# xl-tang3/RCOT

Measured on AMD Instinct MI355X. Metric: 128x128 patches/sec (gen+critic step), higher is better.
Workload: dtype fp32 (exact fp32 MFMA everywhere); 1 GPU; BASELINE configs[1]: Restormer T_net(decoder=True)+F_net(128), denoise_50, RMSprop, paired, B=8/GPU 128x128; global_batch=8, patch=128, parallelism=dp1, gemm_prec=fp32

## Files before the change

include/rcot_hip.h:

```cpp
#ifndef RCOT_HIP_H
#define RCOT_HIP_H
#include <stddef.h>

#ifdef __cplusplus
extern "C" {
#endif

#define RCOT_ABI_VERSION 39

#define RCOT_PREC_FP32 0
#define RCOT_PREC_BF16X3 1
#define RCOT_PREC_BF16X6 2
#define RCOT_PREC_BF16X1 3

int rcot_abi_version(void);
int rcot_debug_nt_coop(int mask);
int rcot_profile_begin(void);
int rcot_profile_end(char* out, int n);
int rcot_last_kernel(char* out, int n);

int rcot_conv1x1_fwd(const float* W, long ldw, const float* X, long sXb, float* Y, long sYb, int B, int Ci, int Co,
                     int N, const float* ln_mu, const float* ln_rs, const float* ln_w, const float* ln_b,
                     const float* R, long sRb, float beta, void* stream);
int rcot_conv1x1_dgrad(const float* W, long ldw, const float* dY, long sdYb, float* dX, long sdXb, int B, int Ci,
// ... 62 lines not shown
int rcot_conv_pcm_merge(const float* dQ, long ldq, float* dX, int B, int C, int H, int W, void* stream);
int rcot_conv_pcm_pack(const float* W, const int* rowoff, const int* koff, int M, int K, void* Apk, void* stream);
int rcot_conv_pcm(const void* Apk, int M, int K, const float* Xp, long ldb, int N, const int* tapoff, int ntaps, const float* bias,
                  float lrelu, const int* colmap, float* Y, long ldy, float* ws, size_t ws_bytes, void* stream);
int rcot_pixel_shuffle(const float* in, float* out, long planes, int H, int W, int mode, void* stream);

int rcot_ln_stats(const float* x, float* mu, float* rs, int B, int C, int N, void* stream);
int rcot_ln_bwd(const float* g, const float* x, const float* mu, const float* rs, const float* w, const float* dres,
                float* dx, float* dw, float* db, int B, int C, int N, void* ws, long ws_bytes, void* stream);
int rcot_ln_bwd_rows(int B, int C, int N);
int rcot_block_param_reduce(const float* part1, const float* part2, int rows, int C, float* gw1, float* gb1, float* gw2,
                            float* gb2, const float* dWo_part, float* gWo, const float* dtemp_part, float* gtemp, int B,
                            int heads, const long long* slab_sets, int n_sets, void* stream);

int rcot_dwconv3x3(const float* x, const float* w, float* y, int B, int C, int H, int W, int flip, void* stream);
int rcot_gdfn_gate_fwd(const float* p, const float* w, float* g, int B, int hid, int H, int W, void* stream);
int rcot_gdfn_gate_bwd(const float* p, const float* w, const float* dg, float* dd, float* dwg, int B, int hid, int H,
                       int W, void* stream);
int rcot_gdfn_bwd(const float* p, const float* w, const float* dg, float* dp, float* dwg, float* dd_scratch, int B, int hid,
                  int H, int W, void* stream);
int rcot_dwconv3x3_wgrad(const float* dy, const float* x, float* dw, int B, int C, int H, int W, void* stream);
int rcot_dwconv3x3_bwd(const float* dy, const float* x, const float* w, float* dx, float* dwg, int B, int C, int H, int W,
                       void* stream);

int rcot_row_sumsq(const float* x, float* out, int B, int R, int N, long sXb, void* stream);
int rcot_attn_softmax(const float* Graw, int S, int ld, const float* sq, const float* temp, float* Gn, float* A, int B,
                      int heads, int c, void* stream);
int rcot_attn_bwd_small(const float* dA, const float* A, const float* Gn, const float* sq, const float* temp,
                        float* dtemp_part, float* Eq, float* EqT, float* Dq, float* Dk, int B, int heads, int c,
                        void* stream);
int rcot_attn_core_fwd(const float* u, long sUb, const float* temp, const float* WoT, long ldwt, float* sq, float* Gn, float* A,
                       float* MfT, long ldm, long sMb, int B, int heads, int c, int N, float* ws, size_t ws_bytes, void* stream);
int rcot_attn_core_bwd(const float* dM, int S, int ldd, const float* Wo, const float* A, const float* Gn, const float* sq,
                       const float* temp, float* Mf, float* dWo_part, float* dtemp_part, float* Eq, float* EqT, float* Dq, float* Dk, int B,
                       int heads, int c, void* stream);
int rcot_attn_rows_bwd(const float* dM, int S, int ldd, const float* Wo, const float* A, const float* Gn, const float* sq,
                       const float* temp, float* Mf, float* dWo_part, float* dtemp_part, float* Eq, float* EqT, float* Dq, float* Dk, int B,
                       int heads, int c, int group_tiles, void* ws, size_t ws_bytes, void* stream);
int rcot_attn_rows_ws_bytes(int B, int heads, int c, int group_tiles);
int rcot_batch_reduce(const float* src, float* dst, int B, long n, float beta, void* stream);

int rcot_lrelu_bwd(const float* dy, const float* a, float* dz, long n, float slope, void* stream);
int rcot_bias_grad(const float* dz, float* db, int B, int C, int P, void* stream);
int rcot_axpby2d(const float* x, long sx, const float* y, long sy, float* out, long so, long rows, long cols, float a,
                 float b, void* stream);
int rcot_fill(float* p, long n, float v, void* stream);
int rcot_lerp(const float* t, const float* f, const float* alpha, float* out, int B, long per, void* stream);
// ... 97 lines not shown
```

rcot_amd/csrc/attn_core.hip:

```cpp
#include <cstdlib>
#include "gemm_core.h"
#include "../../include/rcot_hip.h"

using namespace rcot;

namespace {

template <int CT>
struct AHead {
    static constexpr int cp = 16 * CT;
    static constexpr int c = CT == 2 ? 24 : cp;
    static constexpr int LDA = (cp % 32 == 16) ? cp : cp + 16;
};

template <int CT>
struct AC : AHead<CT> {
    using AHead<CT>::cp;
    using AHead<CT>::c;
    using AHead<CT>::LDA;
    static constexpr int PX = CT == 6 ? 128 : 256;
    static constexpr int Q4 = PX / 4;
    static constexpr int LDQ = PX + 8;
    static constexpr int NW = CT == 6 ? 8 : 4;
    static constexpr int NT = 64 * NW;
// ... 12 lines not shown
__device__ __forceinline__ void fold_prefetch(float (&bfr)[AC<CT>::MTW][AC<CT>::cp / 4], const float* __restrict__ WoT, long ldwt, int h,
                                              int mt0, int mt1) {
    constexpr int cp = AC<CT>::cp, c = AC<CT>::c, NW = AC<CT>::NW, MTW = AC<CT>::MTW;
    const int lane = threadIdx.x & 63, wave = threadIdx.x >> 6;
    const int r16 = lane & 15, kq = lane >> 4;
#pragma unroll
    for (int t = 0; t < MTW; ++t) {
        const int mt = mt0 + wave + NW * t;
        const float* Wl = WoT + ((long)h * c + kq) * ldwt + 16 * mt + r16;
#pragma unroll
        for (int s = 0; s < cp / 4; ++s) bfr[t][s] = (mt < mt1 && 4 * s + kq < c) ? Wl[(long)(4 * s) * ldwt] : 0.f;
    }
}

template <int CT>
__device__ __forceinline__ void attn_tail(float* Gs, const float* sqs, const float (&bfr)[AC<CT>::MTW][AC<CT>::cp / 4], int h, int b,
                                          int heads, const float* __restrict__ temp, float* __restrict__ Gn,
                                          float* __restrict__ A, float* __restrict__ MfT, long ldm, long sMb, int mt0, int mt1,
                                          bool small_out) {
    constexpr int cp = AC<CT>::cp, c = AC<CT>::c, LDA = AC<CT>::LDA, NW = AC<CT>::NW, NT = AC<CT>::NT, MTW = AC<CT>::MTW;
    const int lane = threadIdx.x & 63, wave = threadIdx.x >> 6;
#ifdef AC_NO_TAIL
    if (sMb != -12345) return;
#endif
    const long off = ((long)b * heads + h) * c * c;
    const float tau = temp[h];
    const int grp = threadIdx.x >> 4, gl = threadIdx.x & 15;
    float kn[CT];
#pragma unroll
    for (int t = 0; t < CT; ++t) kn[t] = gl + 16 * t < c ? clamp_norm(sqs[cp + gl + 16 * t]) : 1.f;
#pragma unroll 1
    for (int i = grp; i < cp; i += NT / 16) {
        float* row = Gs + i * LDA;
        const float nq = clamp_norm(sqs[i]);
        float g[CT], e[CT], mx = -INFINITY, sum = 0.f;
#pragma unroll
// ... 11 lines not shown
        }
#pragma unroll
        for (int o = 8; o > 0; o >>= 1) sum += __shfl_xor(sum, o, 64);
        const float inv = i < c ? 1.0f / sum : 0.f;
#pragma unroll
        for (int t = 0; t < CT; ++t) {
            const int j = gl + 16 * t;
            row[j] = e[t] * inv;
            if (small_out && i < c && j < c) {
                Gn[off + i * c + j] = g[t];
                A[off + i * c + j] = e[t] * inv;
            }
        }
    }
    __syncthreads();
    const int r16 = lane & 15, kq = lane >> 4;
    float* Mh = MfT + (long)b * sMb + (long)h * c * ldm;
#pragma unroll
    for (int t = 0; t < MTW; ++t) {
        const int mt = mt0 + wave + NW * t;
        if (mt >= mt1) break;
#pragma unroll 1
        for (int jt = 0; jt < CT; ++jt) {
            f32x4 acc = {0.f, 0.f, 0.f, 0.f};
            const float* Ga = Gs + kq * LDA + 16 * jt + r16;
#pragma unroll
            for (int s = 0; s < cp / 4; ++s) acc = __builtin_amdgcn_mfma_f32_16x16x4f32(Ga[4 * s * LDA], bfr[t][s], acc, 0, 0, 0);
            float* Md = Mh + (long)(16 * jt + 4 * kq) * ldm + 16 * mt + r16;
#pragma unroll
            for (int r = 0; r < 4; ++r)
                if (16 * jt + 4 * kq + r < c) Md[(long)r * ldm] = acc[r];
        }
    }
}

template <int CT>
__global__ __launch_bounds__(AC<CT>::NT) void qk_stats_kernel(const float* __restrict__ u, long sUb, int heads, int N, int pxw,
                                                              float* __restrict__ gpart, float* __restrict__ sqpart,
                                                              const float* __restrict__ temp, const float* __restrict__ WoT, long ldwt,
                                                              float* __restrict__ sq, float* __restrict__ Gn, float* __restrict__ A,
                                                              float* __restrict__ MfT, long ldm, long sMb) {
    using K = AC<CT>;
    constexpr int cp = K::cp, c = K::c, LDA = K::LDA, PX = K::PX, LDQ = K::LDQ, NW = K::NW, NT = K::NT, Q4 = K::Q4, RPP = K::RPP, KQ = K::KQ;
    extern __shared__ __attribute__((aligned(16))) float sm[];
    float* T = sm;
    float* Gs = T + K::TILE;
    float* sqs = Gs + cp * LDA;
    const int tid = threadIdx.x, lane = tid & 63, wave = tid >> 6;
// ... 181 lines not shown
        RCOT_LAUNCH_CHECK();
        return RCOT_OK;
    }
    const int pxw = N == 256 ? 128 : (N > 16384 && N % 2048 == 0) ? 2048 : ((N > 1024 && N % 512 == 0) ? 512 : 256);
    const int S = N / pxw;
    const size_t Z = (size_t)B * heads;
    const size_t need = Z * S * ((size_t)c * c + 2 * c) * sizeof(float);
    if (!ws || ws_bytes < need) return RCOT_EWORKSPACE;
    float* gpart = ws;
    float* sqpart = ws + Z * S * c * c;
    launch_lds<qk_stats_kernel<CT>>(dim3(S, heads, B), dim3(K::NT), K::smem_stats, st, u, sUb, heads, N, pxw, gpart, sqpart, temp, WoT,
                                    ldwt, sq, Gn, A, MfT, ldm, sMb);
    RCOT_LAUNCH_CHECK();
    RCOT_LAUNCH(softmax_fold_kernel<CT>, dim3(ms, heads, B), dim3(K::NT), K::smem_fold, st, gpart, sqpart, S, heads, temp, WoT,
                       ldwt, sq, Gn, A, MfT, ldm, sMb);
    RCOT_LAUNCH_CHECK();
    return RCOT_OK;
}

template <int CT>
struct AB : AHead<CT> {
    using AHead<CT>::cp;
    using AHead<CT>::c;
    using AHead<CT>::LDA;
    static constexpr int LD = cp + 2;
    static constexpr int NW = 4, NT = 256;
    static constexpr int NEL = (cp * cp + NT - 1) / NT;
    static constexpr int Q4 = c / 4;
    static constexpr int NLD = (16 * Q4 + 63) / 64;
    static_assert(NW * 2 * 16 * LD >= cp * LDA, "Gn is staged in the tile region for the tail");
// ... 512 lines not shown
int rcot_attn_core_fwd(const float* u, long sUb, const float* temp, const float* WoT, long ldwt, float* sq, float* Gn, float* A,
                       float* MfT, long ldm, long sMb, int B, int heads, int c, int N, float* ws, size_t ws_bytes, void* stream) {
    if (!u || !temp || !WoT || !sq || !Gn || !A || !MfT || B <= 0 || heads <= 0 || c <= 0 || N <= 0 || B > 65535 || heads > 65535)
        return RCOT_EINVAL;
    const int C = heads * c;
    if ((reinterpret_cast<uintptr_t>(u) & 15) || (sUb & 3) || ldwt < C || ldm < C) return RCOT_EINVAL;
    if ((C % 16) || (N % 256) || N > 65536) return RCOT_EUNSUPPORTED;
    if (N > 4096 && (N % 512)) return RCOT_EUNSUPPORTED;
    hipStream_t st = (hipStream_t)stream;
    if (c == 48) return launch_core_fwd<3>(u, sUb, temp, WoT, ldwt, sq, Gn, A, MfT, ldm, sMb, B, heads, c, N, ws, ws_bytes, st);
    if (c == 96) return launch_core_fwd<6>(u, sUb, temp, WoT, ldwt, sq, Gn, A, MfT, ldm, sMb, B, heads, c, N, ws, ws_bytes, st);
    if (c == 24) return launch_core_fwd<2>(u, sUb, temp, WoT, ldwt, sq, Gn, A, MfT, ldm, sMb, B, heads, c, N, ws, ws_bytes, st);
    return RCOT_EUNSUPPORTED;
}

int rcot_attn_core_bwd(const float* dM, int S, int ldd, const float* Wo, const float* A, const float* Gn, const float* sq,
                       const float* temp, float* Mf, float* dWo_part, float* dtemp_part, float* Eq, float* EqT, float* Dq, float* Dk, int B,
                       int heads, int c, void* stream) {
    if (!dM || !Wo || !A || !Gn || !sq || !temp || !Mf || !dWo_part || !dtemp_part || !Eq || !EqT || !Dq || !Dk || B <= 0 ||
        heads <= 0 || B > 65535 || heads > 65535 || S < 0 || S > 8)
        return RCOT_EINVAL;
    const int C = heads * c;
    if ((C % 16) || (c != 24 && c != 48 && c != 96)) return RCOT_EUNSUPPORTED;
    if (S == 0) ldd = C;
    if (ldd < C || (ldd & 3) || (reinterpret_cast<uintptr_t>(dM) & 15) || (reinterpret_cast<uintptr_t>(Wo) & 15)) return RCOT_EINVAL;
    const long sDs = (long)C * ldd, sDb = (long)(S < 1 ? 1 : S) * sDs;
    hipStream_t st = (hipStream_t)stream;
    if (c == 48) return launch_core_bwd<3>(dM, S, ldd, sDs, sDb, Wo, A, Gn, sq, temp, Mf, dWo_part, dtemp_part, Eq, EqT, Dq, Dk, B, heads, st);
    if (c == 96) return launch_core_bwd<6>(dM, S, ldd, sDs, sDb, Wo, A, Gn, sq, temp, Mf, dWo_part, dtemp_part, Eq, EqT, Dq, Dk, B, heads, st);
    return launch_core_bwd<2>(dM, S, ldd, sDs, sDb, Wo, A, Gn, sq, temp, Mf, dWo_part, dtemp_part, Eq, EqT, Dq, Dk, B, heads, st);
// ... 35 lines not shown
```

rcot_amd/csrc/stencil.hip:

```cpp
#include <type_traits>
#include "common.h"
#include "../../include/rcot_hip.h"

using namespace rcot;

namespace {

struct Row6 { float v[6]; };
struct Patch { Row6 r[6]; };

__device__ __forceinline__ float from_lane_below(float v) {
    return __builtin_bit_cast(float, __builtin_amdgcn_update_dpp(0, __builtin_bit_cast(int, v), 0x138, 0xf, 0xf, true));
}
__device__ __forceinline__ float from_lane_above(float v) {
    return __builtin_bit_cast(float, __builtin_amdgcn_update_dpp(0, __builtin_bit_cast(int, v), 0x130, 0xf, 0xf, true));
}

__device__ __forceinline__ float keep_bits(float v, int mask) {
    return __builtin_bit_cast(float, __builtin_bit_cast(int, v) & mask);
}

__device__ __forceinline__ void load_row6(const float* __restrict__ plane, int H, int W, int y, int x0, Row6& r) {
    if (y < 0 || y >= H) {
#pragma unroll
// ... 100 lines not shown
    const BlockIdx4 b = block4(q, H, W);
    const int c = (int)(b.plane % C);
    Patch r;
    if (NB) {
        PatchRows rows;
        patch_request(x + b.plane * H * W, H, W, b.y0, b.x0, rows);
        patch_land(rows, H, W, b.y0, b.x0, r);
    } else {
        load_patch(x + b.plane * H * W, H, W, b.y0, b.x0, r);
    }
    float o[4][4];
    stencil16<FLIP>(r, w + c * 9, o);
    float* yp = y + b.plane * H * W + (long)b.y0 * W + b.x0;
#pragma unroll
    for (int i = 0; i < 4; ++i) *reinterpret_cast<float4*>(yp + (long)i * W) = make_float4(o[i][0], o[i][1], o[i][2], o[i][3]);
}

template <bool NB>
__global__ __launch_bounds__(256) void gate_fwd_kernel(const float* __restrict__ p, const float* __restrict__ w,
                                                       float* __restrict__ g, long nblocks, int hid, int H, int W) {
    const long q = (long)blockIdx.x * 256 + threadIdx.x;
    if (q >= nblocks) return;
    const BlockIdx4 b = block4(q, H, W);
    const long bi = b.plane / hid;
    const int j = (int)(b.plane - bi * hid);
    const long hw = (long)H * W;
    const float* p1 = p + (bi * 2 * hid + j) * hw;
    Patch r;
    float d1[4][4], d2[4][4];
    if (NB) {
// ... 422 lines not shown
        RCOT_LAUNCH(dwconv_any_kernel, dim3(grid_for(total)), dim3(256), 0, (hipStream_t)stream, x, w, y, total, C, H, W);
        RCOT_LAUNCH_CHECK();
        return RCOT_OK;
    }
    if (!al16(x) || !al16(y)) return RCOT_EINVAL;
    const long nq = (long)B * C * (H >> 2) * (W >> 2);
    const bool nb = nb_lanes_ok(W);
#define RCOT_DW(F, NB_) do { note_kernel("dwconv_kernel<%s, %s>", tf(F), tf(NB_)); RCOT_LAUNCH((dwconv_kernel<F, NB_>), dim3(cdiv(nq, 256)), dim3(256), 0, (hipStream_t)stream, x, w, y, nq, C, H, W); } while (0)
    if (flip) { if (nb) RCOT_DW(true, true); else RCOT_DW(true, false); }
    else { if (nb) RCOT_DW(false, true); else RCOT_DW(false, false); }
#undef RCOT_DW
    RCOT_LAUNCH_CHECK();
    return RCOT_OK;
}

int rcot_gdfn_gate_fwd(const float* p, const float* w, float* g, int B, int hid, int H, int W, void* stream) {
    if (!p || !w || !g || B <= 0 || hid <= 0 || H <= 0 || W <= 0) return RCOT_EINVAL;
    if ((W & 3) || (H & 3)) {
        const long total = (long)B * hid * H * W;
        note_kernel("gate_fwd_any_kernel");
        RCOT_LAUNCH(gate_fwd_any_kernel, dim3(grid_for(total)), dim3(256), 0, (hipStream_t)stream, p, w, g, total, hid, H, W);
        RCOT_LAUNCH_CHECK();
        return RCOT_OK;
    }
    if (!al16(p) || !al16(g)) return RCOT_EINVAL;
    const long nq = (long)B * hid * (H >> 2) * (W >> 2);
    const bool nb = nb_lanes_ok(W);
    note_kernel("gate_fwd_kernel<%s>", tf(nb));
    if (nb)
        RCOT_LAUNCH(gate_fwd_kernel<true>, dim3(cdiv(nq, 256)), dim3(256), 0, (hipStream_t)stream, p, w, g, nq, hid, H, W);
// ... 82 lines not shown
```

rcot_amd/lib.py:

```python
from __future__ import annotations

import ctypes as C
import os

_HERE = os.path.dirname(os.path.abspath(__file__))
ABI_VERSION = 39
PREC_FP32, PREC_BF16X3, PREC_BF16X6, PREC_BF16X1 = 0, 1, 2, 3
SUMSQ_MAX_PARTS, CB_WORDS = 4096, 16
DECIDE_ADAM0, DECIDE_ADAM1, DECIDE_INHERIT = 1, 2, 4
CB_LR, CB_MAX_NORM, CB_NORM, CB_SCALE, CB_STEPS, CB_CLIPPED, CB_SKIPPED, CB_MAX_SEEN, CB_SKIP, CB_T, CB_BC1, CB_BC2 = 0, 1, 2, 3, 4, 5, 6, 7, 8, 9, 11, 13
LIB_PATH = os.environ.get("RCOT_LIB") or os.path.join(_HERE, "librcot_hip.so")


class RcotLibraryError(RuntimeError):
    pass


class RcotKernelError(RuntimeError):
    pass


_f = C.c_void_p
_l = C.c_long
_i = C.c_int
# ... 37 lines not shown
    "rcot_linear_wgrad": [_f, _f, _f, _i, _i, _i, _fl, _f],
    "rcot_conv2d_fwd": [_f, _f, _f, _f, _i, _i, _i, _i, _i, _i, _i, _i, _i, _fl, _i, _f, _f, _fl, _f, _sz, _f],
    "rcot_conv2d_dgrad": [_f, _f, _f, _i, _i, _i, _i, _i, _i, _i, _i, _i, _fl, _f, _fl, _f, _sz, _f],
    "rcot_conv2d_wgrad": [_f, _f, _f, _i, _i, _i, _i, _i, _i, _i, _i, _i, _fl, _f, _sz, _f],
    "rcot_conv_pcm_prep": [_f, _f, _l, _i, _i, _i, _i, _i, _f],
    "rcot_conv_pcm_wgrad": [_f, _f, _l, _i, _i, _i, _i, _f, _fl, _f, _sz, _i, _f],
    "rcot_conv_pcm_merge": [_f, _l, _f, _i, _i, _i, _i, _f],
    "rcot_conv_pcm_pack": [_f, _f, _f, _i, _i, _f, _f],
    "rcot_conv_pcm": [_f, _i, _i, _f, _l, _i, _f, _i, _f, _fl, _f, _f, _l, _f, _sz, _f],
    "rcot_pixel_shuffle": [_f, _f, _l, _i, _i, _i, _f],
    "rcot_ln_stats": [_f, _f, _f, _i, _i, _i, _f],
    "rcot_ln_bwd": [_f, _f, _f, _f, _f, _f, _f, _f, _f, _i, _i, _i, _f, _l, _f],
    "rcot_ln_bwd_rows": [_i, _i, _i],
    "rcot_block_param_reduce": [_f, _f, _i, _i, _f, _f, _f, _f, _f, _f, _f, _f, _i, _i, _f, _i, _f],
    "rcot_dwconv3x3": [_f, _f, _f, _i, _i, _i, _i, _i, _f],
    "rcot_gdfn_gate_fwd": [_f, _f, _f, _i, _i, _i, _i, _f],
    "rcot_gdfn_gate_bwd": [_f, _f, _f, _f, _f, _i, _i, _i, _i, _f],
    "rcot_gdfn_bwd": [_f, _f, _f, _f, _f, _f, _i, _i, _i, _i, _f],
    "rcot_dwconv3x3_wgrad": [_f, _f, _f, _i, _i, _i, _i, _f],
    "rcot_dwconv3x3_bwd": [_f, _f, _f, _f, _f, _i, _i, _i, _i, _f],
    "rcot_row_sumsq": [_f, _f, _i, _i, _i, _l, _f],
    "rcot_attn_softmax": [_f, _i, _i, _f, _f, _f, _f, _i, _i, _i, _f],
    "rcot_attn_bwd_small": [_f, _f, _f, _f, _f, _f, _f, _f, _f, _f, _i, _i, _i, _f],
    "rcot_attn_core_fwd": [_f, _l, _f, _f, _l, _f, _f, _f, _f, _l, _l, _i, _i, _i, _i, _f, _sz, _f],
    "rcot_attn_core_bwd": [_f, _i, _i] + [_f] * 12 + [_i, _i, _i, _f],
    "rcot_attn_rows_bwd": [_f, _i, _i] + [_f] * 12 + [_i, _i, _i, _i, _f, _sz, _f],
    "rcot_attn_rows_ws_bytes": [_i, _i, _i, _i],
    "rcot_batch_reduce": [_f, _f, _i, _l, _fl, _f],
    "rcot_lrelu_bwd": [_f, _f, _f, _l, _fl, _f],
    "rcot_bias_grad": [_f, _f, _i, _i, _i, _f],
    "rcot_axpby2d": [_f, _l, _f, _l, _f, _l, _l, _l, _fl, _fl, _f],
    "rcot_fill": [_f, _l, _fl, _f],
    "rcot_lerp": [_f, _f, _f, _f, _i, _l, _f],
    "rcot_gp_penalty": [_f, _f, _f, _f, _i, _l, _fl, _f],
    "rcot_ot_reduce": [_f, _f, _f, _f, _i, _l, _f],
    "rcot_fft_plan": [_i, _f, _i],
    "rcot_ot_spectrum": [_f, _f, _f, _f, _f, _f, _sz, _i, _i, _i, _f],
    "rcot_ot_grad": [_f, _f, _f, _f, _f, _f, _f, _f, _f, _i, _l, _fl, _fl, _l, _f],
    "rcot_patch_prep": [_f, _f, _i, _i, _i, _i, _i, _i, _fl, C.c_ulonglong, _f, _f, _f],
# ... 78 lines not shown
```

rcot_amd/net_restormer.py:

```python
from __future__ import annotations

from collections import OrderedDict
from typing import Callable, Dict, List, Optional

import numpy as np

import torch

from . import params as P


class ParamStore:

    def __init__(self, be, shapes, live_order: List[str], dead: List[str]):
        self.be = be
        self.shapes = list(shapes)
        self.layout = P.make_layout(shapes, live_order, dead)
        self.flat = be.zeros(self.layout.n_total)
        self.grad = be.zeros(self.layout.n_total)
        self.p: Dict[str, torch.Tensor] = {}
        self.g: Dict[str, torch.Tensor] = {}
        for name, shp in self.shapes:
            o = self.layout.offset[name]
            n = int(np.prod(shp))
# ... 128 lines not shown
        B, _, H, W = x.shape
        N = H * W
        fast = be.kmajor_worth(C, N, B)
        pstats = wmask is None and getattr(be, "stats_ok", None) is not None and be.stats_ok(C, N, B)
        self.out_stats = None
        t = be.empty(B, 3 * C, H, W)
        if in_stats is not None and pstats:
            mu1, rs1 = in_stats
            be.conv1x1_fwd(self.Wqkv, x, t, ln=(mu1, rs1, self.w1, self.b1), packed=self.pk_qkv)
        else:
            mu1, rs1 = be.empty(B, N), be.empty(B, N)
            be.conv1x1_fwd(self.Wqkv, x, t, ln=(mu1, rs1, self.w1, self.b1), packed=self.pk_qkv, ln_compute=True)
        if wmask is not None:
            t[..., wmask:].zero_()
        u = be.empty(B, 3 * C, H, W)
        be.dwconv3x3(t, self.Wdw, u)
        if wmask is not None:
            u[..., wmask:].zero_()
        sq = be.empty(B, 2 * C)
        Q, K, V = self._qkv_views(u)
        Gn, A, MfT = be.empty(B, hd, c, c), be.empty(B, hd, c, c), be.empty(B, C, C)
        if not be.attn_core_fwd(u, self.temp, self.pk_o[0], sq, Gn, A, MfT):
            be.row_sumsq(u[:, :2 * C], sq)
            Graw = be.bmm_nt_slabs(Q, K)
            if Graw is None:
                Graw = be.empty(B, hd, c, c)
                be.bmm_nt(Q, K, Graw)
            be.attn_softmax(Graw, sq, self.temp, Gn, A)
            be.bmm_nn(A, self._woT_heads(B), MfT.view(B, hd, c, C), transA=True)
        y = be.empty(B, C, H, W)
        mu2, rs2 = be.empty(B, N), be.empty(B, N)
        if fast and pstats:
            be.gemm_kmajor_stats(MfT.unsqueeze(1), V, y.view(B, 1, C, N), C, C, x.view(B, 1, C, N), (mu2, rs2))
        elif fast:
            be.gemm_kmajor(MfT.unsqueeze(1), V, y.view(B, 1, C, N), C, C, R=x.view(B, 1, C, N))
        else:
            be.bmm_nn(MfT.unsqueeze(1), V, y.view(B, 1, C, N), transA=True, R=x.view(B, 1, C, N))
# ... 695 lines not shown
```

rcot_amd/ops.py:

```python
from __future__ import annotations

from typing import Optional, Sequence, Tuple

import os
import struct
import sys

import ctypes as C

import torch

from . import lib as _lib

LN = Optional[Tuple[torch.Tensor, torch.Tensor, torch.Tensor, torch.Tensor]]


ctypes_ll = C.c_longlong


def _ptr(t: Optional[torch.Tensor]):
    return None if t is None else t.data_ptr()


def check_patch_rows(rows, P: int, deg_out, clean_out) -> None:
# ... 841 lines not shown
            self._held_gen[g] = self._held + [dWo_part, dtemp_part]
            self._held = []
            self._side_pending = True
            self._gen ^= 1
            return
        if close_block:
            self.side_join()
        launch()

    def dwconv3x3(self, x, w, y, flip: bool = False):
        B, Cc, H, W = x.shape
        assert x.is_contiguous() and y.is_contiguous() and w.is_contiguous()
        _lib.check(self.L.rcot_dwconv3x3(x.data_ptr(), w.data_ptr(), y.data_ptr(), B, Cc, H, W, int(flip), self._st()),
                   "rcot_dwconv3x3")

    def gdfn_gate_fwd(self, p, w, g):
        B, c2, H, W = p.shape
        assert p.is_contiguous() and g.is_contiguous() and w.is_contiguous()
        _lib.check(self.L.rcot_gdfn_gate_fwd(p.data_ptr(), w.data_ptr(), g.data_ptr(), B, c2 // 2, H, W, self._st()),
                   "rcot_gdfn_gate_fwd")

    def gdfn_gate_bwd(self, p, w, dg, dd, dw=None):
        B, c2, H, W = p.shape
        assert p.is_contiguous() and dg.is_contiguous() and dd.is_contiguous() and (dw is None or dw.is_contiguous())
        _lib.check(self.L.rcot_gdfn_gate_bwd(p.data_ptr(), w.data_ptr(), dg.data_ptr(), dd.data_ptr(), _ptr(dw), B, c2 // 2,
                                             H, W, self._st()), "rcot_gdfn_gate_bwd")

    @staticmethod
    def gdfn_bwd_needs_scratch(H: int, W: int) -> bool:
        wq = W // 4
# ... 28 lines not shown
        B, R, N, sx = self._bcn(x, "row_sumsq x")
        assert out.is_contiguous()
        _lib.check(self.L.rcot_row_sumsq(x.data_ptr(), out.data_ptr(), B, R, N, sx, self._st()), "rcot_row_sumsq")

    def attn_softmax(self, Graw, sq, temp, Gn, A):
        B, heads, c, _ = Gn.shape
        for t in (sq, temp, Gn, A):
            assert t.is_contiguous()
        if isinstance(Graw, tuple):
            gp, S, ld = Graw
        else:
            assert Graw.is_contiguous() and tuple(Graw.shape) == tuple(Gn.shape)
            gp, S, ld = Graw.data_ptr(), 0, c
        _lib.check(self.L.rcot_attn_softmax(gp, S, ld, sq.data_ptr(), temp.data_ptr(), Gn.data_ptr(), A.data_ptr(),
                                            B, heads, c, self._st()), "rcot_attn_softmax")

    def attn_core_fwd(self, u, temp, WoT, sq, Gn, A, MfT) -> bool:
        B, heads, c, _ = Gn.shape
        N = u.shape[2] * u.shape[3]
        if N > self.attn_core_maxn:
            return False
        for t in (u, temp, sq, Gn, A, MfT):
            assert t.is_contiguous()
        assert WoT.stride(1) == 1 and tuple(MfT.shape) == (B, heads * c, heads * c) and u.shape[1] == 3 * heads * c
        rc = self.L.rcot_attn_core_fwd(u.data_ptr(), u.stride(0), temp.data_ptr(), WoT.data_ptr(), WoT.stride(0), sq.data_ptr(),
                                       Gn.data_ptr(), A.data_ptr(), MfT.data_ptr(), MfT.stride(1), MfT.stride(0), B, heads, c, N,
                                       self.ws.data_ptr(), self.ws_bytes, self._st())
        if rc == _lib.EUNSUPPORTED:
            return False
        _lib.check(rc, "rcot_attn_core_fwd")
# ... 464 lines not shown
```

rcot_amd/profiling.py:

```python
from __future__ import annotations

import ctypes
from collections import defaultdict
from typing import Dict

import torch

GEMM_OPS = ("gemm_kmajor", "gemm_kmajor_stats", "gemm_kmajor_multi", "conv1x1_fwd", "conv1x1_dgrad", "conv1x1_dgrad_wgrad_slabs", "conv1x1_wgrad", "conv1x1_wgrad_slabs", "bmm_nn", "bmm_nt",
            "bmm_nt_slabs", "linear_fwd", "linear_dgrad",
            "linear_wgrad", "conv2d_fwd", "conv2d_dgrad", "conv2d_wgrad")
OTHER_OPS = ("ln_stats", "ln_bwd", "dwconv3x3", "gdfn_gate_fwd", "gdfn_gate_bwd", "gdfn_bwd", "dwconv3x3_wgrad", "dwconv3x3_bwd", "row_sumsq",
             "attn_softmax", "attn_bwd_small", "batch_reduce", "block_param_reduce", "lrelu_bwd", "bias_grad", "axpby", "fill", "lerp", "gp_penalty",
             "pixel_shuffle", "pack_weight", "ot_reduce", "ot_spectrum", "ot_grad", "rmsprop_step", "adam_step",
             "grad_sumsq", "grad_decide", "rmsprop_step_guarded", "adam_step_guarded")


def _numel(t):
    if not isinstance(t, torch.Tensor):
        return 0
    n = 1
    for sz, st in zip(t.shape, t.stride()):
        if st != 0:
            n *= sz
    return n


# ... 64 lines not shown
            if name == "block_param_reduce" and kw.get("close_block") and not getattr(self.be, "defer_close", False):
                self.be.side_join()
            s.record()
            self._depth += 1
            try:
                r = fn(*a, **kw)
            finally:
                self._depth -= 1
            e.record()
            sym = name
            if self._kname is not None and self._kname(self._kbuf, 192) != seq0:
                sym = self._kbuf.value.decode()
            nbytes = 4.0 * (sum(_numel(t) for t in a) + sum(_numel(t) for t in kw.values()))
            if name == "gemm_kmajor_multi":
                nbytes = 4.0 * sum(_numel(t) for it in a[0] for t in it)
            ln = kw.get("ln")
            if ln is not None:
                nbytes += 4.0 * sum(_numel(t) for t in ln)
            key = name + str(tuple(tuple(t.shape) for t in (a[:4] if name != "gemm_kmajor_multi" else [it[2] for it in a[0]]) if isinstance(t, torch.Tensor)))
            if ln is not None:
                key += "+ln"
            self.records.append((name, s, e, _flops(name, a, kw) if gemm else 0.0, nbytes, key, sym))
            if key not in self._calls:
                self._calls[key] = (fn, a, kw)
            return r
        return timed

    def remove(self):
        for name, fn in self._orig.items():
            setattr(self.be, name, fn)
# ... 69 lines not shown
```

Measured before the change: 108.3 patches/s.

## Fuse q/k row sum-of-squares into dwconv and add softmax+fold path for large MDTA

For large-resolution MDTA layers (where the fused attn_core_fwd path is not used), the depthwise 3x3 conv now also emits per-wave partial sums of squares for the Q and K channels. This removes the separate row_sumsq pass over u. A new softmax_fold entry reduces the slab-split Q·K^T partials and normalizes the rows from those partials. It then applies softmax and folds A with Wo^T, by default as two kernels (per-row softmax, then fold), with an optional single slab-fold kernel. This cuts memory passes and launches, at the cost of extra partial buffers and new code paths.

```diff
diff --git a/include/rcot_hip.h b/include/rcot_hip.h
--- a/include/rcot_hip.h
+++ b/include/rcot_hip.h
@@ -6,7 +6,7 @@
 extern "C" {
 #endif
 
-#define RCOT_ABI_VERSION 39
+#define RCOT_ABI_VERSION 40
 
 #define RCOT_PREC_FP32 0
 #define RCOT_PREC_BF16X3 1
@@ -100,6 +100,7 @@
                             int heads, const long long* slab_sets, int n_sets, void* stream);
 
 int rcot_dwconv3x3(const float* x, const float* w, float* y, int B, int C, int H, int W, int flip, void* stream);
+int rcot_dwconv3x3_sumsq(const float* x, const float* w, float* y, float* sqpart, int B, int C, int H, int W, int R, void* stream);
 int rcot_gdfn_gate_fwd(const float* p, const float* w, float* g, int B, int hid, int H, int W, void* stream);
 int rcot_gdfn_gate_bwd(const float* p, const float* w, const float* dg, float* dd, float* dwg, int B, int hid, int H,
                        int W, void* stream);
@@ -117,6 +118,9 @@
                         void* stream);
 int rcot_attn_core_fwd(const float* u, long sUb, const float* temp, const float* WoT, long ldwt, float* sq, float* Gn, float* A,
                        float* MfT, long ldm, long sMb, int B, int heads, int c, int N, float* ws, size_t ws_bytes, void* stream);
+int rcot_attn_softmax_fold(const float* Graw, int S, int ld, const float* sqpart, int P, const float* temp, const float* WoT, long ldwt,
+                           float* sq, float* Gn, float* A, float* MfT, long ldm, long sMb, int B, int heads, int c, int form,
+                           void* stream);
 int rcot_attn_core_bwd(const float* dM, int S, int ldd, const float* Wo, const float* A, const float* Gn, const float* sq,
                        const float* temp, float* Mf, float* dWo_part, float* dtemp_part, float* Eq, float* EqT, float* Dq, float* Dk, int B,
                        int heads, int c, void* stream);
diff --git a/rcot_amd/csrc/attn_core.hip b/rcot_amd/csrc/attn_core.hip
--- a/rcot_amd/csrc/attn_core.hip
+++ b/rcot_amd/csrc/attn_core.hip
@@ -50,12 +50,36 @@
 }
 
 template <int CT>
+__device__ __forceinline__ void fold_tiles(const float* Gs, const float (&bfr)[AC<CT>::MTW][AC<CT>::cp / 4], int h, int b,
+                                           float* __restrict__ MfT, long ldm, long sMb, int mt0, int mt1) {
+    constexpr int cp = AC<CT>::cp, c = AC<CT>::c, LDA = AC<CT>::LDA, NW = AC<CT>::NW, MTW = AC<CT>::MTW;
+    const int lane = threadIdx.x & 63, wave = threadIdx.x >> 6;
+    const int r16 = lane & 15, kq = lane >> 4;
+    float* Mh = MfT + (long)b * sMb + (long)h * c * ldm;
+#pragma unroll
+    for (int t = 0; t < MTW; ++t) {
+        const int mt = mt0 + wave + NW * t;
+        if (mt >= mt1) break;
+#pragma unroll 1
+        for (int jt = 0; jt < CT; ++jt) {
+            f32x4 acc = {0.f, 0.f, 0.f, 0.f};
+            const float* Ga = Gs + kq * LDA + 16 * jt + r16;
+#pragma unroll
+            for (int s = 0; s < cp / 4; ++s) acc = __builtin_amdgcn_mfma_f32_16x16x4f32(Ga[4 * s * LDA], bfr[t][s], acc, 0, 0, 0);
+            float* Md = Mh + (long)(16 * jt + 4 * kq) * ldm + 16 * mt + r16;
+#pragma unroll
+            for (int r = 0; r < 4; ++r)
+                if (16 * jt + 4 * kq + r < c) Md[(long)r * ldm] = acc[r];
+        }
+    }
+}
+
+template <int CT>
 __device__ __forceinline__ void attn_tail(float* Gs, const float* sqs, const float (&bfr)[AC<CT>::MTW][AC<CT>::cp / 4], int h, int b,
                                           int heads, const float* __restrict__ temp, float* __restrict__ Gn,
                                           float* __restrict__ A, float* __restrict__ MfT, long ldm, long sMb, int mt0, int mt1,
                                           bool small_out) {
-    constexpr int cp = AC<CT>::cp, c = AC<CT>::c, LDA = AC<CT>::LDA, NW = AC<CT>::NW, NT = AC<CT>::NT, MTW = AC<CT>::MTW;
-    const int lane = threadIdx.x & 63, wave = threadIdx.x >> 6;
+    constexpr int cp = AC<CT>::cp, c = AC<CT>::c, LDA = AC<CT>::LDA, NT = AC<CT>::NT;
 #ifdef AC_NO_TAIL
     if (sMb != -12345) return;
 #endif
@@ -97,24 +121,7 @@
         }
     }
     __syncthreads();
-    const int r16 = lane & 15, kq = lane >> 4;
-    float* Mh = MfT + (long)b * sMb + (long)h * c * ldm;
-#pragma unroll
-    for (int t = 0; t < MTW; ++t) {
-        const int mt = mt0 + wave + NW * t;
-        if (mt >= mt1) break;
-#pragma unroll 1
-        for (int jt = 0; jt < CT; ++jt) {
-            f32x4 acc = {0.f, 0.f, 0.f, 0.f};
-            const float* Ga = Gs + kq * LDA + 16 * jt + r16;
-#pragma unroll
-            for (int s = 0; s < cp / 4; ++s) acc = __builtin_amdgcn_mfma_f32_16x16x4f32(Ga[4 * s * LDA], bfr[t][s], acc, 0, 0, 0);
-            float* Md = Mh + (long)(16 * jt + 4 * kq) * ldm + 16 * mt + r16;
-#pragma unroll
-            for (int r = 0; r < 4; ++r)
-                if (16 * jt + 4 * kq + r < c) Md[(long)r * ldm] = acc[r];
-        }
-    }
+    fold_tiles<CT>(Gs, bfr, h, b, MfT, ldm, sMb, mt0, mt1);
 }
 
 template <int CT>
@@ -326,6 +333,181 @@
     RCOT_LAUNCH_CHECK();
     RCOT_LAUNCH(softmax_fold_kernel<CT>, dim3(ms, heads, B), dim3(K::NT), K::smem_fold, st, gpart, sqpart, S, heads, temp, WoT,
                        ldwt, sq, Gn, A, MfT, ldm, sMb);
+    RCOT_LAUNCH_CHECK();
+    return RCOT_OK;
+}
+
+template <int CT>
+struct ASF : AC<CT> {
+    using AC<CT>::c;
+    using AC<CT>::cp;
+    using AC<CT>::NW;
+    static constexpr int Q4 = c / 4;
+    static constexpr int NP = c * Q4;
+    static constexpr int PG = CT == 6 ? 4 : 1;
+    static constexpr int SG = NW / PG;
+    static constexpr int PP = NP / (64 * PG);
+    static_assert(cp == c && PP * 64 * PG == NP && SG * PG == NW, "piece map");
+};
+
+__device__ __forceinline__ float norm_from_parts(const float* __restrict__ sqpart, long row, int P) {
+    const float* sp = sqpart + row * P;
+    float t = 0.f;
+#pragma unroll 8
+    for (int p = 0; p < P; ++p) t += sp[p];
+    return t;
+}
+
+template <int CT>
+__global__ __launch_bounds__(AC<CT>::NT) void attn_slab_fold_kernel(const float* __restrict__ Graw, int S, int ld,
+                                                                    const float* __restrict__ sqpart, int P, int heads,
+                                                                    const float* __restrict__ temp, const float* __restrict__ WoT,
+                                                                    long ldwt, float* __restrict__ sq, float* __restrict__ Gn,
+                                                                    float* __restrict__ A, float* __restrict__ MfT, long ldm, long sMb) {
+    using K = ASF<CT>;
+    constexpr int cp = K::cp, c = K::c, LDA = K::LDA, NT = K::NT, Q4 = K::Q4, PG = K::PG, SG = K::SG, PP = K::PP;
+    extern __shared__ __attribute__((aligned(16))) float sm[];
+    float* Gs = sm;
+    float* sqs = Gs + cp * LDA;
+    const int tid = threadIdx.x, lane = tid & 63, wave = tid >> 6;
+    const int ms = blockIdx.x, h = blockIdx.y, b = blockIdx.z;
+    const int C = heads * c;
+    const int mt0 = ms * K::MT_WG, mt1 = min(C / 16, mt0 + K::MT_WG);
+    float bfr[K::MTW][cp / 4];
+    fold_prefetch<CT>(bfr, WoT, ldwt, h, mt0, mt1);
+    for (int r = tid; r < 2 * c; r += NT) {
+        const long row = (long)b * 2 * C + (r < c ? h * c + r : C + h * c + r - c);
+        const float t = norm_from_parts(sqpart, row, P);
+        sqs[r < c ? r : cp + r - c] = t;
+        if (ms == 0) sq[row] = t;
+    }
+    const long slab = (long)c * ld;
+    const float* gp = Graw + ((long)b * heads + h) * S * slab;
+    const int pg = wave % PG, sg = wave / PG;
+    f32x4 a[PP];
+#pragma unroll
+    for (int k = 0; k < PP; ++k) a[k] = f32x4{0.f, 0.f, 0.f, 0.f};
+#pragma unroll 1
+    for (int s = sg; s < S; s += 2 * SG) {
+        const bool two = s + SG < S;
+        f32x4 v0[PP], v1[PP];
+#pragma unroll
+        for (int k = 0; k < PP; ++k) {
+            const int p = (pg * PP + k) * 64 + lane, i = p / Q4, c4 = p - i * Q4;
+            const float* src = gp + (long)s * slab + (long)i * ld + 4 * c4;
+            v0[k] = *reinterpret_cast<const f32x4*>(src);
+            v1[k] = two ? *reinterpret_cast<const f32x4*>(src + (long)SG * slab) : f32x4{0.f, 0.f, 0.f, 0.f};
+        }
+#pragma unroll
+        for (int k = 0; k < PP; ++k) {
+            a[k] += v0[k];
+            a[k] += v1[k];
+        }
+    }
+#pragma unroll 1
+    for (int rd = 0; rd < SG; ++rd) {
+        if (sg == rd) {
+#pragma unroll
+            for (int k = 0; k < PP; ++k) {
+                const int p = (pg * PP + k) * 64 + lane, i = p / Q4, c4 = p - i * Q4;
+                f32x4* d = reinterpret_cast<f32x4*>(Gs + i * LDA + 4 * c4);
+                *d = rd == 0 ? a[k] : *d + a[k];
+            }
+        }
+        __syncthreads();
+    }
+    attn_tail<CT>(Gs, sqs, bfr, h, b, heads, temp, Gn, A, MfT, ldm, sMb, mt0, mt1, ms == 0);
+}
+
+__global__ __launch_bounds__(256) void attn_softmax_parts_kernel(const float* __restrict__ Graw, int S, int ld,
+                                                                 const float* __restrict__ sqpart, int P,
+                                                                 const float* __restrict__ temp, float* __restrict__ sq,
+                                                                 float* __restrict__ Gn, float* __restrict__ A, int heads, int c) {
+    __shared__ float part[4][128];
+    __shared__ float nsq[129];
+    const int i = blockIdx.x, h = blockIdx.y, b = blockIdx.z;
+    const int C = heads * c;
+    const int tid = threadIdx.x, wave = tid >> 6, lane = tid & 63;
+    if (tid < c || tid == 128) {
+        const long row = (long)b * 2 * C + (tid < c ? C + h * c + tid : h * c + i);
+        const float t = norm_from_parts(sqpart, row, P);
+        nsq[tid] = t;
+        if (tid == 128 || i == 0) sq[row] = t;
+    }
+    const long off = ((long)b * heads + h) * c * c;
+    const float tau = temp[h];
+    const bool a0 = lane < c, a1 = lane + 64 < c;
+    const long slab = (long)c * ld;
+    const float* w = Graw + ((long)b * heads + h) * S * slab + (long)i * ld + lane;
+    float q0[4] = {0.f, 0.f, 0.f, 0.f}, q1[4] = {0.f, 0.f, 0.f, 0.f};
+    int s = wave;
+    for (; s + 12 < S; s += 16) {
+#pragma unroll
+        for (int u = 0; u < 4; ++u) {
+            if (a0) q0[u] += w[(long)(s + 4 * u) * slab];
+            if (a1) q1[u] += w[(long)(s + 4 * u) * slab + 64];
+        }
+    }
+    for (; s < S; s += 4) {
+        if (a0) q0[0] += w[(long)s * slab];
+        if (a1) q1[0] += w[(long)s * slab + 64];
+    }
+    part[wave][lane] = (q0[0] + q0[1]) + (q0[2] + q0[3]);
+    part[wave][lane + 64] = (q1[0] + q1[1]) + (q1[2] + q1[3]);
+    __syncthreads();
+    if (wave != 0) return;
+    const float r0 = (part[0][lane] + part[1][lane]) + (part[2][lane] + part[3][lane]);
+    const float r1 = (part[0][lane + 64] + part[1][lane + 64]) + (part[2][lane + 64] + part[3][lane + 64]);
+    const float k0 = a0 ? clamp_norm(nsq[lane]) : 1.f, k1 = a1 ? clamp_norm(nsq[lane + 64]) : 1.f;
+    const float nq = clamp_norm(nsq[128]);
+    const float g0 = a0 ? r0 / (nq * k0) : 0.f;
+    const float g1 = a1 ? r1 / (nq * k1) : 0.f;
+    const float v0 = a0 ? g0 * tau : -INFINITY, v1 = a1 ? g1 * tau : -INFINITY;
+    const float mx = wave_max(fmaxf(v0, v1));
+    const float e0 = a0 ? expf(v0 - mx) : 0.f, e1 = a1 ? expf(v1 - mx) : 0.f;
+    const float inv = 1.0f / wave_sum(e0 + e1);
+    if (a0) { Gn[off + i * c + lane] = g0; A[off + i * c + lane] = e0 * inv; }
+    if (a1) { Gn[off + i * c + lane + 64] = g1; A[off + i * c + lane + 64] = e1 * inv; }
+}
+
+template <int CT>
+__global__ __launch_bounds__(AC<CT>::NT) void attn_fold_kernel(const float* __restrict__ A, int heads, const float* __restrict__ WoT,
+                                                               long ldwt, float* __restrict__ MfT, long ldm, long sMb) {
+    using K = ASF<CT>;
+    constexpr int cp = K::cp, c = K::c, LDA = K::LDA, NT = K::NT, Q4 = K::Q4, NP = K::NP;
+    extern __shared__ __attribute__((aligned(16))) float sm[];
+    float* Gs = sm;
+    const int ms = blockIdx.x, h = blockIdx.y, b = blockIdx.z;
+    const int C = heads * c;
+    const int mt0 = ms * K::MT_WG, mt1 = min(C / 16, mt0 + K::MT_WG);
+    float bfr[K::MTW][cp / 4];
+    fold_prefetch<CT>(bfr, WoT, ldwt, h, mt0, mt1);
+    const float* Az = A + ((long)b * heads + h) * c * c;
+    for (int p = threadIdx.x; p < NP; p += NT) {
+        const int i = p / Q4, c4 = p - i * Q4;
+        *reinterpret_cast<f32x4*>(Gs + i * LDA + 4 * c4) = *reinterpret_cast<const f32x4*>(Az + 4 * p);
+    }
+    __syncthreads();
+    fold_tiles<CT>(Gs, bfr, h, b, MfT, ldm, sMb, mt0, mt1);
+}
+
+template <int CT>
+int launch_softmax_fold(const float* Graw, int S, int ld, const float* sqpart, int P, const float* temp, const float* WoT, long ldwt,
+                        float* sq, float* Gn, float* A, float* MfT, long ldm, long sMb, int B, int heads, int c, int form,
+                        hipStream_t st) {
+    using K = AC<CT>;
+    const int ms = cdiv(heads * c / 16, K::MT_WG);
+    if (form == 1) {
+        note_kernel("attn_slab_fold_kernel<%d>", CT);
+        RCOT_LAUNCH(attn_slab_fold_kernel<CT>, dim3(ms, heads, B), dim3(K::NT), K::smem_fold, st, Graw, S, ld, sqpart, P, heads, temp,
+                    WoT, ldwt, sq, Gn, A, MfT, ldm, sMb);
+        RCOT_LAUNCH_CHECK();
+        return RCOT_OK;
+    }
+    RCOT_LAUNCH(attn_softmax_parts_kernel, dim3(c, heads, B), dim3(256), 0, st, Graw, S, ld, sqpart, P, temp, sq, Gn, A, heads, c);
+    RCOT_LAUNCH_CHECK();
+    note_kernel("attn_fold_kernel<%d>", CT);
+    RCOT_LAUNCH(attn_fold_kernel<CT>, dim3(ms, heads, B), dim3(K::NT), K::smem_fold, st, A, heads, WoT, ldwt, MfT, ldm, sMb);
     RCOT_LAUNCH_CHECK();
     return RCOT_OK;
 }
@@ -868,6 +1050,22 @@
     return RCOT_EUNSUPPORTED;
 }
 
+int rcot_attn_softmax_fold(const float* Graw, int S, int ld, const float* sqpart, int P, const float* temp, const float* WoT, long ldwt,
+                           float* sq, float* Gn, float* A, float* MfT, long ldm, long sMb, int B, int heads, int c, int form,
+                           void* stream) {
+    if (!Graw || !sqpart || !temp || !WoT || !sq || !Gn || !A || !MfT || B <= 0 || heads <= 0 || B > 65535 || heads > 65535 || S < 0 ||
+        P <= 0 || form < 0 || form > 2)
+        return RCOT_EINVAL;
+    if (c != 48 && c != 96) return RCOT_EUNSUPPORTED;
+    const int C = heads * c;
+    if (S == 0) { S = 1; ld = c; }
+    if (ld < c || (ld & 3) || !al16(Graw) || !al16(A) || ldwt < C || ldm < C) return RCOT_EINVAL;
+    if (form == 0) form = 2;
+    hipStream_t st = (hipStream_t)stream;
+    if (c == 48) return launch_softmax_fold<3>(Graw, S, ld, sqpart, P, temp, WoT, ldwt, sq, Gn, A, MfT, ldm, sMb, B, heads, c, form, st);
+    return launch_softmax_fold<6>(Graw, S, ld, sqpart, P, temp, WoT, ldwt, sq, Gn, A, MfT, ldm, sMb, B, heads, c, form, st);
+}
+
 int rcot_attn_core_bwd(const float* dM, int S, int ldd, const float* Wo, const float* A, const float* Gn, const float* sq,
                        const float* temp, float* Mf, float* dWo_part, float* dtemp_part, float* Eq, float* EqT, float* Dq, float* Dk, int B,
                        int heads, int c, void* stream) {
diff --git a/rcot_amd/csrc/stencil.hip b/rcot_amd/csrc/stencil.hip
--- a/rcot_amd/csrc/stencil.hip
+++ b/rcot_amd/csrc/stencil.hip
@@ -138,6 +138,51 @@
     float* yp = y + b.plane * H * W + (long)b.y0 * W + b.x0;
 #pragma unroll
     for (int i = 0; i < 4; ++i) *reinterpret_cast<float4*>(yp + (long)i * W) = make_float4(o[i][0], o[i][1], o[i][2], o[i][3]);
+}
+
+__device__ __forceinline__ float wave_sum_dpp(float v) {
+    v += __builtin_bit_cast(float, __builtin_amdgcn_update_dpp(0, __builtin_bit_cast(int, v), 0x128, 0xf, 0xf, false));
+    v += __builtin_bit_cast(float, __builtin_amdgcn_update_dpp(0, __builtin_bit_cast(int, v), 0x124, 0xf, 0xf, false));
+    v += __builtin_bit_cast(float, __builtin_amdgcn_update_dpp(0, __builtin_bit_cast(int, v), 0x122, 0xf, 0xf, false));
+    v += __builtin_bit_cast(float, __builtin_amdgcn_update_dpp(0, __builtin_bit_cast(int, v), 0x121, 0xf, 0xf, false));
+    v += __shfl_xor(v, 16, 64);
+    v += __shfl_xor(v, 32, 64);
+    return v;
+}
+
+template <bool NB>
+__global__ __launch_bounds__(256) void dwconv_sumsq_kernel(const float* __restrict__ x, const float* __restrict__ w,
+                                                           float* __restrict__ y, float* __restrict__ sqpart, long nblocks, int C,
+                                                           int R, int P, int H, int W) {
+    const long q = (long)blockIdx.x * 256 + threadIdx.x;
+    if (q >= nblocks) return;
+    const BlockIdx4 b = block4(q, H, W);
+    const long img = b.plane / C;
+    const int c = (int)(b.plane - img * C);
+    Patch r;
+    if (NB) {
+        PatchRows rows;
+        patch_request(x + b.plane * H * W, H, W, b.y0, b.x0, rows);
+        patch_land(rows, H, W, b.y0, b.x0, r);
+    } else {
+        load_patch(x + b.plane * H * W, H, W, b.y0, b.x0, r);
+    }
+    float o[4][4];
+    stencil16<false>(r, w + c * 9, o);
+    float* yp = y + b.plane * H * W + (long)b.y0 * W + b.x0;
+#pragma unroll
+    for (int i = 0; i < 4; ++i) *reinterpret_cast<float4*>(yp + (long)i * W) = make_float4(o[i][0], o[i][1], o[i][2], o[i][3]);
+    if (c >= R) return;
+    float s[4];
+#pragma unroll
+    for (int i = 0; i < 4; ++i) {
+        s[i] = o[i][0] * o[i][0];
+#pragma unroll
+        for (int j = 1; j < 4; ++j) s[i] = fmaf(o[i][j], o[i][j], s[i]);
+    }
+    const float t = wave_sum_dpp((s[0] + s[1]) + (s[2] + s[3]));
+    const int wv = (int)((q - b.plane * (long)(H >> 2) * (W >> 2)) >> 6);
+    if ((threadIdx.x & 63) == 0) sqpart[(img * R + c) * P + wv] = t;
 }
 
 template <bool NB>
@@ -590,6 +635,24 @@
     return RCOT_OK;
 }
 
+int rcot_dwconv3x3_sumsq(const float* x, const float* w, float* y, float* sqpart, int B, int C, int H, int W, int R, void* stream) {
+    if (!x || !w || !y || !sqpart || B <= 0 || C <= 0 || H <= 0 || W <= 0 || R <= 0 || R > C) return RCOT_EINVAL;
+    const long per = (long)(H >> 2) * (W >> 2);
+    if ((W & 3) || (H & 3) || (per & 63) || per / 64 > 0x7fffffffL) return RCOT_EUNSUPPORTED;
+    if (!al16(x) || !al16(y)) return RCOT_EINVAL;
+    const long nq = (long)B * C * per;
+    const int P = (int)(per / 64);
+    if (nb_lanes_ok(W)) {
+        note_kernel("dwconv_sumsq_kernel<true>");
+        RCOT_LAUNCH(dwconv_sumsq_kernel<true>, dim3(cdiv(nq, 256)), dim3(256), 0, (hipStream_t)stream, x, w, y, sqpart, nq, C, R, P, H, W);
+    } else {
+        note_kernel("dwconv_sumsq_kernel<false>");
+        RCOT_LAUNCH(dwconv_sumsq_kernel<false>, dim3(cdiv(nq, 256)), dim3(256), 0, (hipStream_t)stream, x, w, y, sqpart, nq, C, R, P, H, W);
+    }
+    RCOT_LAUNCH_CHECK();
+    return RCOT_OK;
+}
+
 int rcot_gdfn_gate_fwd(const float* p, const float* w, float* g, int B, int hid, int H, int W, void* stream) {
     if (!p || !w || !g || B <= 0 || hid <= 0 || H <= 0 || W <= 0) return RCOT_EINVAL;
     if ((W & 3) || (H & 3)) {
diff --git a/rcot_amd/lib.py b/rcot_amd/lib.py
--- a/rcot_amd/lib.py
+++ b/rcot_amd/lib.py
@@ -4,7 +4,7 @@
 import os
 
 _HERE = os.path.dirname(os.path.abspath(__file__))
-ABI_VERSION = 39
+ABI_VERSION = 40
 PREC_FP32, PREC_BF16X3, PREC_BF16X6, PREC_BF16X1 = 0, 1, 2, 3
 SUMSQ_MAX_PARTS, CB_WORDS = 4096, 16
 DECIDE_ADAM0, DECIDE_ADAM1, DECIDE_INHERIT = 1, 2, 4
@@ -75,6 +75,7 @@
     "rcot_ln_bwd_rows": [_i, _i, _i],
     "rcot_block_param_reduce": [_f, _f, _i, _i, _f, _f, _f, _f, _f, _f, _f, _f, _i, _i, _f, _i, _f],
     "rcot_dwconv3x3": [_f, _f, _f, _i, _i, _i, _i, _i, _f],
+    "rcot_dwconv3x3_sumsq": [_f, _f, _f, _f, _i, _i, _i, _i, _i, _f],
     "rcot_gdfn_gate_fwd": [_f, _f, _f, _i, _i, _i, _i, _f],
     "rcot_gdfn_gate_bwd": [_f, _f, _f, _f, _f, _i, _i, _i, _i, _f],
     "rcot_gdfn_bwd": [_f, _f, _f, _f, _f, _f, _i, _i, _i, _i, _f],
@@ -84,6 +85,7 @@
     "rcot_attn_softmax": [_f, _i, _i, _f, _f, _f, _f, _i, _i, _i, _f],
     "rcot_attn_bwd_small": [_f, _f, _f, _f, _f, _f, _f, _f, _f, _f, _i, _i, _i, _f],
     "rcot_attn_core_fwd": [_f, _l, _f, _f, _l, _f, _f, _f, _f, _l, _l, _i, _i, _i, _i, _f, _sz, _f],
+    "rcot_attn_softmax_fold": [_f, _i, _i, _f, _i, _f, _f, _l, _f, _f, _f, _f, _l, _l, _i, _i, _i, _i, _f],
     "rcot_attn_core_bwd": [_f, _i, _i] + [_f] * 12 + [_i, _i, _i, _f],
     "rcot_attn_rows_bwd": [_f, _i, _i] + [_f] * 12 + [_i, _i, _i, _i, _f, _sz, _f],
     "rcot_attn_rows_ws_bytes": [_i, _i, _i, _i],
diff --git a/rcot_amd/net_restormer.py b/rcot_amd/net_restormer.py
--- a/rcot_amd/net_restormer.py
+++ b/rcot_amd/net_restormer.py
@@ -166,13 +166,23 @@
         if wmask is not None:
             t[..., wmask:].zero_()
         u = be.empty(B, 3 * C, H, W)
-        be.dwconv3x3(t, self.Wdw, u)
+        route = getattr(be, "mdta_large_route", None)
+        form = route(c, hd, H, W) if route is not None and wmask is None else 0
+        sqp = be.dwconv3x3_sumsq(t, self.Wdw, u, 2 * C) if form else None
+        if sqp is None:
+            be.dwconv3x3(t, self.Wdw, u)
         if wmask is not None:
             u[..., wmask:].zero_()
         sq = be.empty(B, 2 * C)
         Q, K, V = self._qkv_views(u)
         Gn, A, MfT = be.empty(B, hd, c, c), be.empty(B, hd, c, c), be.empty(B, C, C)
-        if not be.attn_core_fwd(u, self.temp, self.pk_o[0], sq, Gn, A, MfT):
+        if sqp is not None:
+            Graw = be.bmm_nt_slabs(Q, K)
+            if Graw is None:
+                Graw = be.empty(B, hd, c, c)
+                be.bmm_nt(Q, K, Graw)
+            be.attn_softmax_fold(Graw, sqp, self.temp, self.pk_o[0], sq, Gn, A, MfT, form)
+        elif not be.attn_core_fwd(u, self.temp, self.pk_o[0], sq, Gn, A, MfT):
             be.row_sumsq(u[:, :2 * C], sq)
             Graw = be.bmm_nt_slabs(Q, K)
             if Graw is None:
diff --git a/rcot_amd/ops.py b/rcot_amd/ops.py
--- a/rcot_amd/ops.py
+++ b/rcot_amd/ops.py
@@ -879,6 +879,18 @@
         _lib.check(self.L.rcot_dwconv3x3(x.data_ptr(), w.data_ptr(), y.data_ptr(), B, Cc, H, W, int(flip), self._st()),
                    "rcot_dwconv3x3")
 
+    def dwconv3x3_sumsq(self, x, w, y, R: int):
+        B, Cc, H, W = x.shape
+        assert x.is_contiguous() and y.is_contiguous() and w.is_contiguous() and 0 < R <= Cc
+        if H % 4 or W % 4 or ((H // 4) * (W // 4)) % 64:
+            return None
+        sqpart = self.empty(B, R, (H // 4) * (W // 4) // 64)
+        rc = self.L.rcot_dwconv3x3_sumsq(x.data_ptr(), w.data_ptr(), y.data_ptr(), sqpart.data_ptr(), B, Cc, H, W, R, self._st())
+        if rc == _lib.EUNSUPPORTED:
+            return None
+        _lib.check(rc, "rcot_dwconv3x3_sumsq")
+        return sqpart
+
     def gdfn_gate_fwd(self, p, w, g):
         B, c2, H, W = p.shape
         assert p.is_contiguous() and g.is_contiguous() and w.is_contiguous()
@@ -937,6 +949,31 @@
             gp, S, ld = Graw.data_ptr(), 0, c
         _lib.check(self.L.rcot_attn_softmax(gp, S, ld, sq.data_ptr(), temp.data_ptr(), Gn.data_ptr(), A.data_ptr(),
                                             B, heads, c, self._st()), "rcot_attn_softmax")
+
+    mdta_large = "auto"
+
+    def mdta_large_route(self, c: int, heads: int, H: int, W: int) -> int:
+        if self.mdta_large == "off" or c not in (48, 96) or H * W <= self.attn_core_maxn:
+            return 0
+        if H % 4 or W % 4 or ((H // 4) * (W // 4)) % 64:
+            return 0
+        if self.mdta_large != "auto":
+            return {"one": 1, "two": 2}[self.mdta_large]
+        return 2
+
+    def attn_softmax_fold(self, Graw, sqpart, temp, WoT, sq, Gn, A, MfT, form: int = 0):
+        B, heads, c, _ = Gn.shape
+        for t in (sqpart, temp, sq, Gn, A, MfT):
+            assert t.is_contiguous()
+        assert WoT.stride(1) == 1 and tuple(MfT.shape) == (B, heads * c, heads * c) and tuple(sqpart.shape[:2]) == (B, 2 * heads * c)
+        if isinstance(Graw, tuple):
+            gp, S, ld = Graw
+        else:
+            assert Graw.is_contiguous() and tuple(Graw.shape) == tuple(Gn.shape)
+            gp, S, ld = Graw.data_ptr(), 0, c
+        _lib.check(self.L.rcot_attn_softmax_fold(gp, S, ld, sqpart.data_ptr(), sqpart.shape[2], temp.data_ptr(), WoT.data_ptr(),
+                                                 WoT.stride(0), sq.data_ptr(), Gn.data_ptr(), A.data_ptr(), MfT.data_ptr(),
+                                                 MfT.stride(1), MfT.stride(0), B, heads, c, form, self._st()), "rcot_attn_softmax_fold")
 
     def attn_core_fwd(self, u, temp, WoT, sq, Gn, A, MfT) -> bool:
         B, heads, c, _ = Gn.shape
diff --git a/rcot_amd/profiling.py b/rcot_amd/profiling.py
--- a/rcot_amd/profiling.py
+++ b/rcot_amd/profiling.py
@@ -9,7 +9,7 @@
 GEMM_OPS = ("gemm_kmajor", "gemm_kmajor_stats", "gemm_kmajor_multi", "conv1x1_fwd", "conv1x1_dgrad", "conv1x1_dgrad_wgrad_slabs", "conv1x1_wgrad", "conv1x1_wgrad_slabs", "bmm_nn", "bmm_nt",
             "bmm_nt_slabs", "linear_fwd", "linear_dgrad",
             "linear_wgrad", "conv2d_fwd", "conv2d_dgrad", "conv2d_wgrad")
-OTHER_OPS = ("ln_stats", "ln_bwd", "dwconv3x3", "gdfn_gate_fwd", "gdfn_gate_bwd", "gdfn_bwd", "dwconv3x3_wgrad", "dwconv3x3_bwd", "row_sumsq",
+OTHER_OPS = ("ln_stats", "ln_bwd", "dwconv3x3", "dwconv3x3_sumsq", "attn_softmax_fold", "gdfn_gate_fwd", "gdfn_gate_bwd", "gdfn_bwd", "dwconv3x3_wgrad", "dwconv3x3_bwd", "row_sumsq",
              "attn_softmax", "attn_bwd_small", "batch_reduce", "block_param_reduce", "lrelu_bwd", "bias_grad", "axpby", "fill", "lerp", "gp_penalty",
              "pixel_shuffle", "pack_weight", "ot_reduce", "ot_spectrum", "ot_grad", "rmsprop_step", "adam_step",
              "grad_sumsq", "grad_decide", "rmsprop_step_guarded", "adam_step_guarded")
@@ -104,6 +104,10 @@
             nbytes = 4.0 * (sum(_numel(t) for t in a) + sum(_numel(t) for t in kw.values()))
             if name == "gemm_kmajor_multi":
                 nbytes = 4.0 * sum(_numel(t) for it in a[0] for t in it)
+            if name == "dwconv3x3_sumsq":
+                nbytes += 4.0 * _numel(r)
+            if name == "attn_softmax_fold" and not isinstance(a[0], torch.Tensor):
+                nbytes += 4.0 * _numel(a[5])
             ln = kw.get("ln")
             if ln is not None:
                 nbytes += 4.0 * sum(_numel(t) for t in ln)
```

Result: no change. 108.7 patches/s (median of 6 runs) (+0.4%).
